# kjyv/FloBaRoID

Measured on AMD Instinct MI355X. Metric: regressor samples/s (fused regressor->Gram pass) + TSQR TFLOP/s, WALK-MAN 31-DOF float-base, higher is better.
Workload: dtype f64

## Files before the change

### flobaroid_amd/csrc/fbr_gram64.h

```cpp
#pragma once
#define FBR_G64_SWZ(c) (2 * ((c) & 15))
#include <algorithm>
#include <type_traits>
#include <utility>

#include "fbr_kinid.h"

struct FbrGram64Tile {
    int col[FBR_TILE];
    std::vector<int> path;
    int friction = 0;
    int lo = 0, hi = 0;
};

struct FbrGram64 {
    int NT = 0;
    int NF = 0;
    int nlev = 0, fb = 0, flev = 0, ntr = 0, maxact = 0, npw = 0, wpb = 8;
    long blk_doubles = 0;
    std::vector<int> trow;
    std::vector<int> slab;
    int nstage = 0, base_stages = 0;
    std::vector<int> stage_lev;
    std::vector<int> lev_begin;
// ... 661 lines not shown
        put(a, b, l[0], l[1], h[0], h[1]);
    }
    __device__ __forceinline__ double get8(double a) const { return dpp<0x128>(a); }
    __device__ __forceinline__ double get7(double a) const { return dpp<0x141>(a); }
    __device__ __forceinline__ double get2(double a) const { return dpp<0x4E>(a); }
    __device__ __forceinline__ double get1(double a) const { return dpp<0xB1>(a); }
    __device__ __forceinline__ double live0(bool live, double a) const { return live ? a : 0.0; }
    __device__ __forceinline__ double bit8(double a, double b) const { return (lane & 8) ? b : a; }
    __device__ __forceinline__ double zero() const { return 0.0; }
};

struct DevGram64 {
    int NT, nlev, maxact, npieces, nstage;
    long blk_doubles;
    const int *slab, *lev_begin, *pieces, *wmeta, *stage_lev;
    const int *runs;
};

template <int MAXD, bool HASW, int KR = 1>
__global__ __launch_bounds__(64 * FBR_KINWRITE_PARTS, MAXD <= 10 ? 2 : 1) void fbr_kinimg_kernel(DevModel m, DevKinId p, DevKinWrite wr, long S, long blk_doubles,
                                                                              const double *__restrict__ q, const double *__restrict__ dq,
                                                                              const double *__restrict__ ddq, const double *__restrict__ bv,
                                                                              const double *__restrict__ ba, const double *__restrict__ rpy,
                                                                              const double *__restrict__ rhs, const double *__restrict__ wts,
                                                                              double *__restrict__ scratch, double *__restrict__ mom,
                                                                              const double *__restrict__ sign)
{
    extern __shared__ __attribute__((aligned(16))) double smem[];
    const int lane = threadIdx.x & 63, part = __builtin_amdgcn_readfirstlane(threadIdx.x >> 6), nth = blockDim.x, tid = threadIdx.x;
    const int n = m.n, ldn = p.ldn, ldw = m.rows | 1, rows = m.rows;
    double *sq = smem, *sdq = sq + 64 * ldn, *sddq = sdq + 64 * ldn, *sw = sddq + 64 * ldn;
    double *st = sw + (HASW ? 64 * ldw : 0);
    double *scr = scratch + ((long)blockIdx.x * wr.nparts + part) * p.nslots * FBR_LINK_REC * 64 + lane;
    double *mo = mom ? mom + (long)blockIdx.x * (KR * wr.cols + KR * (KR + 1) / 2) : nullptr;
    const bool domom = KR > 1 || wr.k != 0;
    const FbrMomLanesDev mx{lane};
    const long Sg = wr.group_samples > 0 ? wr.group_samples : S, bpg = (Sg + 63) >> 6;
    const long nblk = (S / Sg) * bpg;
    const fbr_clong_ptr cdst = (fbr_clong_ptr)(unsigned long)wr.dst;
    const __attribute__((address_space(1))) int *glcol = (const __attribute__((address_space(1))) int *)(unsigned long)wr.lanecol + (long)part * m.L * 64 + lane;
    for (long blk = blockIdx.x; blk < nblk; blk += gridDim.x) {
        const long grp = blk / bpg, lb = blk - grp * bpg;
        const long base = grp * Sg + (lb << 6);
        const int valid = (int)min(64L, Sg - (lb << 6));
        __syncthreads();
        {
            const long off = base * n;
            const int cnt = valid * n;
            int sr = tid / n, dc = tid - sr * n;
            const int ds = nth / n, dd = nth - ds * n;
            for (int i = tid; i < cnt; i += nth) {
                const double a = q[off + i], b = dq[off + i], c = ddq[off + i];
                sq[sr * ldn + dc] = a;
                sdq[sr * ldn + dc] = b;
                sddq[sr * ldn + dc] = c;
                sr += ds;
                dc += dd;
                if (dc >= n) {
                    dc -= n;
                    sr++;
                }
            }
            if (HASW || wr.k) {
                const int cw = valid * rows;
                int wr_ = tid / rows, wc = tid - wr_ * rows;
                const int es = nth / rows, ed = nth - es * rows;
                for (int i = tid; i < cw; i += nth) {
                    const double wv = HASW ? wts[base * rows + i] : 1.0;
                    if (HASW) sw[wr_ * ldw + wc] = wv;
                    if constexpr (KR == 1) {
                        if (wr.k) st[wr_ * ldw + wc] = wv * wv * rhs[base * rows + i];
                    } else {
#pragma unroll
                        for (int r = 0; r < KR; r++) st[r * 64 * ldw + wr_ * ldw + wc] = wv * wv * rhs[(base * rows + i) * KR + r];
                    }
                    wr_ += es;
                    wc += ed;
                    if (wc >= rows) {
                        wc -= rows;
                        wr_++;
                    }
                }
            }
        }
        __syncthreads();
        const int ls = min(lane, valid - 1);
        const long s = base + ls;
        const bool live = lane < valid;
        const double *mysq = sq + ls * ldn, *mysdq = sdq + ls * ldn, *mysddq = sddq + ls * ldn, *myw = sw + ls * ldw, *myt = st + ls * ldw;
        const long slot_off = blk * blk_doubles + (long)(lane >> 5) * 512;
        const int s31 = lane & 31;
        auto state = [&](int d, double &a, double &b, double &c) {
            a = mysq[d];
            b = mysdq[d];
            c = mysddq[d];
        };
        auto basest = [&](double *v6, double *a6, double *e3) {
            for (int i = 0; i < 6; i++) {
                v6[i] = bv[s * 6 + i];
                a6[i] = ba[s * 6 + i];
            }
            for (int i = 0; i < 3; i++) e3[i] = rpy[s * 3 + i];
        };
        auto save = [&](int b, int i, double v) { scr[(b * FBR_LINK_REC + i) * 64] = v; };
        auto load = [&](int b, int i) { return scr[(b * FBR_LINK_REC + i) * 64]; };
        auto consts = [&](int l, double *rR, double *rp, double *ax) {
            const fbr_cdouble_ptr cR = (fbr_cdouble_ptr)(unsigned long)m.restR, cp = (fbr_cdouble_ptr)(unsigned long)m.restp,
                                  ca = (fbr_cdouble_ptr)(unsigned long)m.axis;
            for (int i = 0; i < 9; i++) rR[i] = cR[9 * l + i];
            for (int i = 0; i < 3; i++) {
                rp[i] = cp[3 * l + i];
                ax[i] = ca[3 * l + i];
            }
        };
        const unsigned vlane = (unsigned)(((unsigned long)slot_off + (unsigned long)s31) << 3);
        auto link = [&](int l, int depth, const double *rec, const double (*Sst)[6], const int *lvd, double *F) {
            (void)F;
            if (wr.base_only) depth = 0;
            if (wr.none && ((fbr_cint_ptr)(unsigned long)wr.none)[(long)part * m.L + l]) return;
            int mycol = -1;
            if (domom) mycol = glcol[l * 64];
            __builtin_amdgcn_s_waitcnt(0x0F70);
            double macc = 0.0;
            auto mom_sum = [&](auto g0c, auto ngc, auto p0c, auto nqc, const double *v, int r) {
                constexpr int G0 = decltype(g0c)::value, NG = decltype(ngc)::value, P0 = decltype(p0c)::value, NQ = decltype(nqc)::value;
                double u[NG];
#pragma unroll
                for (int i = 0; i < NG; i++) u[i] = (G0 + i >= P0 && G0 + i < P0 + NQ) ? v[G0 + i - P0] : 0.0;
                const double sum = fbr_mom_lanes_sum<NG>(u, live, mx);
                if (G0 == 0 ? (lane & 15) == 6 * r : (lane & 7) == 1 + 6 * r) macc += sum;
            };
            long d10[10], dF[4];
#pragma unroll
            for (int pp = 0; pp < 10; pp++) d10[pp] = cdst[((long)part * m.L + l) * FBR_G64_WORDS + pp];
#pragma unroll
            for (int pp = 0; pp < 4; pp++) dF[pp] = cdst[((long)part * m.L + l) * FBR_G64_WORDS + 10 + pp];
            auto ft_of = [&](int ro, double *F) {
#pragma unroll
                for (int i = 0; i < 6; i++)
                    if (i < m.fb) F[i] = myt[ro + i];
#pragma unroll
                for (int j = 0; j < MAXD; j++)
                    if (j < depth) {
                        const double tj = myt[ro + m.fb + lvd[j]];
#pragma unroll
                        for (int i = 0; i < 6; i++) F[i] += Sst[j][i] * tj;
                    }
            };
            double Ft[6] = {0.0, 0.0, 0.0, 0.0, 0.0, 0.0};
            if constexpr (KR == 1) {
                if (wr.k) {
#pragma unroll
                    for (int i = 0; i < 6; i++)
                        if (i < m.fb) Ft[i] = myt[i];
#pragma unroll
                    for (int j = 0; j < MAXD; j++)
                        if (j < depth) {
                            const double tj = myt[m.fb + lvd[j]];
#pragma unroll
                            for (int i = 0; i < 6; i++) Ft[i] += Sst[j][i] * tj;
                        }
                }
            }
            auto ft_group = [&](int r, double *F) {
                int ro = r * 64 * ldw;
                asm volatile("" : "+v"(ro));
#pragma unroll
                for (int i = 0; i < 6; i++) F[i] = 0.0;
                ft_of(ro, F);
// ... 72 lines not shown
                if (!domom || any == 0) return;
                double v[NQ];
                if constexpr (KR == 1) {
#pragma unroll
                    for (int qq = 0; qq < NQ; qq++) v[qq] = Ft[3] * nB[qq][0] + Ft[4] * nB[qq][1] + Ft[5] * nB[qq][2];
                    mom_sum(integral_constant<int, 4>{}, integral_constant<int, 6>{}, integral_constant<int, 4 + Q0>{}, nqc, v, 0);
                } else {
#pragma unroll
                    for (int r = 0; r < KR; r++) {
                        double F[6];
                        ft_group(r, F);
#pragma unroll
                        for (int qq = 0; qq < NQ; qq++) v[qq] = F[3] * nB[qq][0] + F[4] * nB[qq][1] + F[5] * nB[qq][2];
                        mom_sum(integral_constant<int, 4>{}, integral_constant<int, 6>{}, integral_constant<int, 4 + Q0>{}, nqc, v, r);
                    }
                }
            };
            if constexpr (MAXD > 8 && MAXD <= 10) {
                full_group(integral_constant<int, 0>{}, integral_constant<int, 2>{});
                full_group(integral_constant<int, 2>{}, integral_constant<int, 2>{});
                moment_group(integral_constant<int, 0>{}, integral_constant<int, 3>{});
                moment_group(integral_constant<int, 3>{}, integral_constant<int, 3>{});
            } else {
                full_group(integral_constant<int, 0>{}, integral_constant<int, 4>{});
                moment_group(integral_constant<int, 0>{}, integral_constant<int, 6>{});
            }
            const int nfr = wr.cols > wr.ninert ? (wr.cols - wr.ninert) / n : 0;
            const int dj = nfr ? m.dof[l] : -1;
            if (dj >= 0 && depth > 0) {
                const fbr_cint_ptr cfr = (fbr_cint_ptr)(unsigned long)(wr.lcol10 + (long)wr.nparts * 10 * m.L + ((long)part * m.L + l) * FBR_G64_FRIC);
#pragma unroll
                for (int pf = 0; pf < FBR_G64_FRIC; pf++)
                    if (pf < nfr) {
                        const long dfw = cdst[((long)part * m.L + l) * FBR_G64_WORDS + 14 + pf];
                        if (dfw == 0) continue;
                        const int c = cfr[pf];
                        const double fv = fbr_friction_value(m.coldesc[c].z, mysdq[dj], sign ? sign[s * n + dj] : 0.0, m.stribeck);
                        store(dfw, m.fb + depth - 1, HASW ? fv * myw[m.fb + dj] : fv);
                        if (!domom) continue;
#pragma unroll
                        for (int r = 0; r < KR; r++) {
                            const double v = fv * myt[r * 64 * ldw + m.fb + dj], sum = fbr_mom_lanes_sum<1>(&v, live, mx);
                            if (lane == fbr_gram64_mom_fric_lane(pf, r)) macc = sum;
                        }
                    }
            }
            if (domom && mycol >= 0 && (KR > 1 || mycol < (1 << FBR_G64_LANECOL_RHS)))
                unsafeAtomicAdd(mo + (mycol >> FBR_G64_LANECOL_RHS) * wr.cols + (mycol & ((1 << FBR_G64_LANECOL_RHS) - 1)), macc);
        };
        auto emit = [&](int, double) {};
        {
            fbr_kinid_lane<MAXD, false>(wr.part_nsteps[part], p.maxlvl, p.steps + wr.part_step0[part] * FBR_KINID_STEP, p.endflush, m.floating, m.g, m.fb,
                                        state, basest, save, load, link, emit, consts);
            if constexpr (KR == 1) {
                if (wr.k && part == wr.nparts - 1) {
                    double tt = 0.0;
                    for (int r = 0; r < rows; r++) {
                        const double wv = HASW ? myw[r] : 1.0, tv = rhs[s * rows + r] * wv;
                        tt += tv * tv;
                    }
                    const double sum = fbr_mom_lanes_sum<1>(&tt, live, mx);
                    if (lane == 0) unsafeAtomicAdd(mo + wr.cols, sum);
                }
            } else if (part == wr.nparts - 1) {
                double tt[KR * (KR + 1) / 2];
#pragma unroll
                for (int e = 0; e < KR * (KR + 1) / 2; e++) tt[e] = 0.0;
// ... 266 lines not shown
```

### flobaroid_amd/csrc/fbr_gram_api.hip

```cpp
#define FBR_KERNELS_GRAM
#include "fbr_internal.h"

static int get_deal(GramHolder *h, int wpg, GramHolder::Deal *out, bool base_only = false)
{
    const int key = wpg | (base_only ? 1 << 24 : 0);
    auto it = h->deals.find(key);
    if (it != h->deals.end()) {
        *out = it->second;
        return FBR_OK;
    }
    const std::vector<int> n = fbr_gram_deal(h->prog, wpg, base_only);
    std::vector<int2> tab;
    std::vector<int> begin(h->prog.T + 1, 0), given(h->prog.T, 0);
    for (int p = 0; p < h->prog.T; p++) begin[p + 1] = begin[p] + n[p];
    while ((int)tab.size() < begin[h->prog.T])
        for (int p = 0; p < h->prog.T; p++)
            if (given[p] < n[p]) tab.push_back(make_int2(p, given[p]++ | (n[p] << 16)));
    GramHolder::Deal d;
    int rc;
    if ((rc = upload(h->pool, tab, &d.tab))) return rc;
    if ((rc = upload(h->pool, begin, &d.begin))) return rc;
    h->deals[key] = d;
    *out = d;
    return FBR_OK;
// ... 250 lines not shown
{
    if (h->g64_state) return FBR_OK;
    h->g64_state = -1;
    const FbrHostModel &hm = m->hm;
    if (m->kinid.nsteps <= 0 || !fbr_gram64_build(hm, h->prog, h->g64, m->opt.gram_force_tiles != 0, m->opt.gram_lane_waves >= 16,
                                                         (int)m->opt.gram_lane_tiling))
        return FBR_OK;
    FbrGram64 &g = h->g64;
    if (fbr_gram64_lds_bytes(g) > FBR_G64_LDS_MAX) return FBR_OK;
    if (gram64_plds(hm, h->prog.k, true) > 160 * 1024) return FBR_OK;
    if (!fbr_gram64_build_producer(hm, g, h->g64p, m->opt.gram_lane_parts_cut != 0, h->prog.k)) return FBR_OK;
    std::vector<int> wgbegin{0, 0};
    int rc;
    if ((rc = upload(h->pool, g.slab, &h->d64_slab)) || (rc = upload(h->pool, g.lev_begin, &h->d64_levb)) || (rc = upload(h->pool, g.pieces, &h->d64_pieces)) ||
        (rc = upload(h->pool, g.wmeta, &h->d64_wmeta)) || (rc = upload(h->pool, h->g64p.lcol, &h->d64_lcol)) ||
        (rc = upload(h->pool, fbr_gram64_lane_columns(h->g64p, hm.L), &h->d64_lanecol)) ||
        (rc = upload(h->pool, h->g64p.steps, &h->d64_steps)) || (rc = upload(h->pool, h->g64p.none, &h->d64_none)) ||
        (rc = upload(h->pool, g.slot_tiles, &h->d64_slot_tiles)) || (rc = upload(h->pool, g.tilecol, &h->d64_tilecol)) ||
        (rc = upload(h->pool, g.stage_lev, &h->d64_stagelev)) || (!g.runs.empty() && (rc = upload(h->pool, g.runs, &h->d64_runs))))
        return rc;
    h->g64_state = 1;
    return FBR_OK;
}

static int gram64_serves(fbr_model *m, GramHolder *h, int k, bool *serves)
{
    *serves = false;
    if (!m->opt.gram_lane || k > FBR_G64_MAXK || (k > 0 && !h->moments)) return FBR_OK;
    if (int rc = get_gram64(m, h)) return rc;
    *serves = h->g64_state == 1;
    return FBR_OK;
}

static long gram64_chunk_blocks(const FbrGram64 &g) { return std::max<long>(1, (long)((size_t)3 * 1024 * 1024 * 1024 / ((size_t)g.blk_doubles * 8))); }

static int gram64_wg_table(GramHolder *h, int wgs, const int **out)
{
    auto it = h->d64_wb.find(wgs);
    if (it == h->d64_wb.end()) {
        std::vector<int> wb{0, wgs};
        const int *dwb = nullptr;
        if (int rc = upload(h->pool, wb, &dwb)) return rc;
        it = h->d64_wb.emplace(wgs, dwb).first;
    }
    *out = it->second;
    return FBR_OK;
}

static int gram64_ensure_images(fbr_model *m, GramHolder *h, long chb)
{
    const FbrGram64 &g = h->g64;
    int rc;
    if (chb <= h->img64_blocks) return FBR_OK;
    for (int b = 0; b < 2; b++) {
        if ((rc = h->img64[b].ensure((size_t)chb * g.blk_doubles * sizeof(double)))) return rc;
        HIPCHK(hipMemsetAsync(h->img64[b].p, 0, h->img64[b].bytes, m->stream));
        std::vector<long long> dst(h->g64p.rel.size(), 0);
        for (size_t i = 0; i < dst.size(); i++)
            if (h->g64p.rel[i]) dst[i] = (long long)(uintptr_t)h->img64[b].p + (h->g64p.rel[i] & ~(1LL << 62));
        if ((rc = h->dst64[b].ensure(dst.size() * sizeof(long long)))) return rc;
        HIPCHK(hipMemcpyAsync(h->dst64[b].p, dst.data(), dst.size() * sizeof(long long), hipMemcpyHostToDevice, m->stream));
        HIPCHK(hipStreamSynchronize(m->stream));
    }
    h->img64_blocks = chb;
    return FBR_OK;
}

template <class F> static auto kinimg_by_depth(const fbr_model *m, F &&f) { return fbr_by_depth<4, 8, 10, 12, FBR_KINID_MAXD>(m->kinid.maxlvl, f); }

struct Gram64Launch {
    DevKinId kp;
    int pgrid_max;
    DevGram64 dg;
    void (*gk)(DevGram64, long, const double *, double *, int);
    size_t glds;
    int vnpw;
};
static int gram64_setup(fbr_model *m, GramHolder *h, bool base_only, Gram64Launch *L)
{
    const FbrGram64 &g = h->g64;
    L->kp = kinid_params(m, 0, h->g64p.nslots, h->d64_steps);
    L->pgrid_max = kinimg_by_depth(m, [](auto D) { return D <= 10 ? 2 : 1; }) * m->num_cus;
    if (int rc = h->scr64.ensure((size_t)L->pgrid_max * h->g64p.nparts * std::max(h->g64p.nslots, 1) * FBR_LINK_REC * 64 * sizeof(double))) return rc;
    DevGram64 &dg = L->dg;
    dg.NT = g.NT + g.NF;
    dg.nlev = g.nlev;
    dg.maxact = g.maxact;
    dg.npieces = (int)g.pieces.size() / 2;
    dg.blk_doubles = g.blk_doubles;
    dg.slab = h->d64_slab;
    dg.lev_begin = h->d64_levb;
    dg.pieces = h->d64_pieces;
    dg.wmeta = h->d64_wmeta;
    dg.nstage = base_only ? g.base_stages : g.nstage;
    dg.stage_lev = h->d64_stagelev;
    dg.runs = g.runs.empty() ? nullptr : h->d64_runs;
    L->gk = g.wpb == 16 ? fbr_gram64_kernel<10, 16>
            : g.npw == 10   ? fbr_gram64_kernel<10, 8>
            : g.runs.empty() ? fbr_gram64_kernel<FBR_ONE_SEGW * FBR_ONE_NSEG, 8> : fbr_gram64_kernel<FBR_ONE_SEGW * FBR_ONE_NSEG, 8, true>;
    L->glds = fbr_gram64_lds_bytes(g);
    L->vnpw = g.npw * (g.wpb / 8);
    HIPCHK(hipFuncSetAttribute((const void *)L->gk, hipFuncAttributeMaxDynamicSharedMemorySize, (int)L->glds));
    return FBR_OK;
}

static DevKinWrite gram64_kinwrite(const fbr_model *m, const GramHolder *h, int b, int k, bool has_w, bool base_only, long group_samples)
{
    DevKinWrite kw{};
    kw.lcol10 = h->d64_lcol;
    kw.lanecol = h->d64_lanecol;
    kw.none = m->opt.gram_lane_skip_unowned != 0 ? h->d64_none : nullptr;
    kw.dst = (const long *)h->dst64[b].p;
    kw.ninert = m->hm.ninert;
    kw.cols = m->hm.cols;
    kw.k = k;
    kw.has_w = has_w ? 1 : 0;
    kw.flev = h->g64.flev;
    kw.base_only = base_only ? 1 : 0;
    kw.group_samples = group_samples;
    kw.nparts = h->g64p.nparts;
    for (int pq = 0; pq < FBR_KINWRITE_PARTS; pq++) {
        kw.part_nsteps[pq] = h->g64p.nsteps[pq];
        kw.part_step0[pq] = h->g64p.step0[pq];
    }
    return kw;
}

static int gram64_produce(fbr_model *m, GramHolder *h, const Gram64Launch &L, const DevKinWrite &kw, int pblocks, size_t plds, long cs,
                          const DevStates &d, long so, const double *rhs, int k, const double *w, double *mom)
{
    const FbrHostModel &hm = m->hm;
    return kinimg_by_depth(m, [&](auto D) -> int {
        const auto kernel = k == 2 ? (kw.has_w ? fbr_kinimg_kernel<D, true, 2> : fbr_kinimg_kernel<D, false, 2>)
                                   : (kw.has_w ? fbr_kinimg_kernel<D, true> : fbr_kinimg_kernel<D, false>);
        HIPCHK(hipFuncSetAttribute((const void *)kernel, hipFuncAttributeMaxDynamicSharedMemorySize, (int)plds));
        hipLaunchKernelGGL(kernel, dim3(pblocks), dim3(64 * h->g64p.nparts), plds, m->stream, m->dm, L.kp, kw, cs, h->g64.blk_doubles, d.q + so * hm.n,
                           d.dq + so * hm.n, d.ddq + so * hm.n, d.bv ? d.bv + so * 6 : nullptr, d.ba ? d.ba + so * 6 : nullptr,
                           d.rpy ? d.rpy + so * 3 : nullptr, rhs ? rhs + (size_t)so * hm.rows * k : nullptr, w ? w + (size_t)so * hm.rows : nullptr,
                           h->scr64.as<double>(), mom, d.sign ? d.sign + so * hm.n : nullptr);
        HIPCHK(hipGetLastError());
        return FBR_OK;
    });
}

static int gram64_reduce(fbr_model *m, GramHolder *h, const Gram64Launch &L, int wpg, const int *wg_begin, int ng, double *G)
// ... 30 lines not shown
        if (int rc = m->st_chunk[b].ensure(std::max<size_t>(1, (size_t)samples * per) * sizeof(double))) return rc;
    return FBR_OK;
}
static int stage_chunk(fbr_model *m, const DevStates &d, const double *rhs, int k, const double *w, long s0, long cs, int b, hipStream_t cps,
                       DevStates *dc, const double **crhs, const double **cw)
{
    const FbrHostModel &hm = m->hm;
    double *p = m->st_chunk[b].as<double>();
    auto put = [&](const double *src, size_t per, const double **dst) -> int {
        *dst = nullptr;
        if (!src || per == 0) return FBR_OK;
        HIPCHK(hipMemcpyAsync(p, src + (size_t)s0 * per, (size_t)cs * per * sizeof(double), hipMemcpyHostToDevice, cps));
        *dst = p;
        p += (size_t)cs * per;
        return FBR_OK;
    };
    *dc = d;
    int rc;
    if ((rc = put(d.q, hm.n, &dc->q)) || (rc = put(d.dq, hm.n, &dc->dq)) || (rc = put(d.ddq, hm.n, &dc->ddq)) || (rc = put(d.bv, 6, &dc->bv)) ||
        (rc = put(d.ba, 6, &dc->ba)) || (rc = put(d.rpy, 3, &dc->rpy)) || (rc = put(d.sign, hm.n, &dc->sign)) ||
        (rc = put(rhs, (size_t)hm.rows * k, crhs)) || (rc = put(w, hm.rows, cw)))
        return rc;
    return FBR_OK;
}

static int gram64_pass(fbr_model *m, GramHolder *h, const DevStates &d, const double *drhs, const double *dw, int k, double *G, bool base_only,
                       bool h2d_chunked)
{
    const FbrHostModel &hm = m->hm;
    const FbrGram64 &g = h->g64;
    const long S = d.S;
    int rc;
    const long nblocks = (S + 63) / 64;
    long chb = gram64_chunk_blocks(g);
    if (h2d_chunked) chb = std::min<long>(chb, 7L * m->num_cus);
    if (m->opt.chunk_samples >= 1) chb = std::min(gram64_chunk_blocks(g), std::max<long>(1, ((long)m->opt.chunk_samples + 63) / 64));
    chb = std::min(nblocks, chb);
    if (chb < nblocks && chb > m->num_cus) chb = chb / m->num_cus * m->num_cus;
    Gram64Launch L;
    if ((rc = gram64_setup(m, h, base_only, &L))) return rc;
    long last_blocks = 0;
    if (m->opt.gram_lane_chunk_rounds != 0 && !h2d_chunked && m->opt.chunk_samples < 1 && chb < nblocks && chb >= m->num_cus) {
        const FbrGram64ChunkPlan cp = fbr_gram64_chunk_plan(nblocks, gram64_chunk_blocks(g), m->num_cus, L.pgrid_max, 1);
        chb = cp.chb;
        last_blocks = cp.last_cap;
    }
    long chs = chb * 64;
    if (m->opt.chunk_samples >= 1) chs = std::min(chs, (long)m->opt.chunk_samples);
    const long last_s = last_blocks > 0 ? last_blocks * 64 : chs;
    auto chunk_len = [&](long s0) { return S - s0 <= last_s ? S - s0 : chs; };
    if ((rc = gram64_ensure_images(m, h, std::min(nblocks, std::max(chb, last_blocks))))) return rc;
    const size_t plds = gram64_plds(hm, k, dw != nullptr);
    const int pblocks = (int)std::min<long>(chb, (long)L.pgrid_max);
    const int gwgs = (int)std::min<long>(chb, (long)m->num_cus);
    if (k) {
        if ((rc = h->mom64.ensure((size_t)L.pgrid_max * fbr_gram64_mom_count(hm.cols, k) * sizeof(double)))) return rc;
        HIPCHK(hipMemsetAsync(h->mom64.p, 0, (size_t)pblocks * fbr_gram64_mom_count(hm.cols, k) * sizeof(double), m->stream));
    }
    if ((rc = m->partial.ensure((size_t)m->num_cus * g.wpb * g.npw * 256 * sizeof(double)))) return rc;
    int launches = 0, first_wgs = 0;
    if (h2d_chunked) {
        if ((rc = ensure_stage_buffers(m, d, k, dw, chs, 2)) || (rc = ensure_copy_stream(m))) return rc;
        HIPCHK(hipEventRecord(m->ev_fork, m->stream));
    }
    struct Staged {
        DevStates dc;
        long o;
        const double *rhs, *w;
    };
    auto stage = [&](long c, Staged &out) -> int {
        const long s0 = c * chs, cs = chunk_len(s0);
        const int b = (int)(c & 1);
        out = {d, s0, drhs, dw};
        if (!h2d_chunked) return FBR_OK;
        HIPCHK(hipStreamWaitEvent(m->copy, m->ev_pack_rec[b] ? m->ev_pack[b] : m->ev_fork, 0));
        ProfScope ps(m, FBR_PROF_H2D, m->copy);
        if (int r3 = stage_chunk(m, d, drhs, k, dw, s0, cs, b, m->copy, &out.dc, &out.rhs, &out.w)) return r3;
        out.o = 0;
        HIPCHK(hipEventRecord(m->ev_h2d[b], m->copy));
        return FBR_OK;
    };
    Staged cur, nxt;
    if (S > 0 && (rc = stage(0, nxt))) return rc;
    for (long s0 = 0, cs = 0; s0 < S; s0 += cs, launches++) {
        cs = chunk_len(s0);
        const long nb = (cs + 63) / 64;
        const int b = launches & 1;
        cur = nxt;
        if (s0 + cs < S && (rc = stage(launches + 1, nxt))) return rc;
        if (h2d_chunked) HIPCHK(hipStreamWaitEvent(m->stream, m->ev_h2d[b], 0));
        {
            ProfScope ps(m, FBR_PROF_PACK);
            if ((rc = gram64_produce(m, h, L, gram64_kinwrite(m, h, b, k, dw != nullptr, base_only, 0), pblocks, plds, cs, cur.dc, cur.o, cur.rhs, k,
                                     cur.w, k ? h->mom64.as<double>() : nullptr)))
                return rc;
            if (cs & 63) {
                hipLaunchKernelGGL(fbr_gram64_tail_zero_kernel, dim3(16, 1), dim3(256), 0, m->stream, h->img64[b].as<double>(), g.blk_doubles, nb, g.ntr, (int)(cs & 63));
                HIPCHK(hipGetLastError());
            }
            if (h2d_chunked) {
                HIPCHK(hipEventRecord(m->ev_pack[b], m->stream));
                m->ev_pack_rec[b] = true;
            }
        }
        const int wgs = (int)std::min<long>(nb, (long)gwgs);
        if (launches == 0) first_wgs = wgs;
        if (wgs > first_wgs) {
            set_err("internal: Gram launch wider than the first one of the call");
            return FBR_E_INVALID;
        }
        {
            ProfScope ps(m, FBR_PROF_GRAM);
            hipLaunchKernelGGL(L.gk, dim3(first_wgs), dim3(g.wpb * 64), L.glds, m->stream, L.dg, nb, h->img64[b].as<double>(), m->partial.as<double>(),
                               launches > 0 ? 1 : 0);
            HIPCHK(hipGetLastError());
        }
    }
    if (launches > 0) {
        ProfScope ps(m, FBR_PROF_REDUCE);
        const int *wgb = nullptr;
        if ((rc = gram64_wg_table(h, first_wgs, &wgb)) || (rc = gram64_reduce(m, h, L, first_wgs, wgb, 1, G))) return rc;
        if (k) {
            hipLaunchKernelGGL(fbr_gram64_mom_reduce_kernel, dim3((fbr_gram64_mom_count(hm.cols, k) + 3) / 4), dim3(256), 0, m->stream, hm.cols, k, pblocks,
                               h->mom64.as<double>(), G);
            HIPCHK(hipGetLastError());
        }
    }
    return FBR_OK;
}

static int gram64_grouped_pass(fbr_model *m, GramHolder *h, const DevStates &d, const double *dw, double *G, int ngroups)
{
    const FbrHostModel &hm = m->hm;
    const FbrGram64 &g = h->g64;
    const long S = d.S, Sg = S / ngroups, bpg = (Sg + 63) / 64;
    const int Pa = hm.cols;
    int rc;
    const int gpc = (int)std::min<long>(std::min(ngroups, 32768), std::max<long>(1, gram64_chunk_blocks(g) / bpg));
    if ((rc = gram64_ensure_images(m, h, (long)gpc * bpg))) return rc;
    const int wpg = (int)std::max<long>(1, std::min<long>(bpg, (long)m->num_cus / std::min(gpc, ngroups)));
    Gram64Launch L;
    if ((rc = gram64_setup(m, h, false, &L))) return rc;
    const size_t plds = gram64_plds(hm, 0, dw != nullptr);
    if ((rc = m->partial.ensure((size_t)gpc * wpg * g.wpb * g.npw * 256 * sizeof(double)))) return rc;
    const int *wgb = nullptr;
    if ((rc = gram64_wg_table(h, wpg, &wgb))) return rc;
    for (int g0 = 0, launches = 0; g0 < ngroups; g0 += gpc, launches++) {
        const int ng = std::min(gpc, ngroups - g0), b = launches & 1;
        const long s0 = (long)g0 * Sg, cs = (long)ng * Sg, nb = (long)ng * bpg;
        {
            ProfScope ps(m, FBR_PROF_PACK);
            if ((rc = gram64_produce(m, h, L, gram64_kinwrite(m, h, b, 0, dw != nullptr, false, Sg), (int)std::min<long>(nb, (long)L.pgrid_max), plds, cs,
                                     d, s0, nullptr, 0, dw, nullptr)))
                return rc;
            if (Sg & 63) {
                hipLaunchKernelGGL(fbr_gram64_tail_zero_kernel, dim3(16, ng), dim3(256), 0, m->stream, h->img64[b].as<double>(), g.blk_doubles, bpg, g.ntr, (int)(Sg & 63));
                HIPCHK(hipGetLastError());
            }
        }
        {
            ProfScope ps(m, FBR_PROF_GRAM);
            hipLaunchKernelGGL(L.gk, dim3(wpg, ng), dim3(g.wpb * 64), L.glds, m->stream, L.dg, bpg, h->img64[b].as<double>(), m->partial.as<double>(), 0);
            HIPCHK(hipGetLastError());
        }
        {
            ProfScope ps(m, FBR_PROF_REDUCE);
            if ((rc = gram64_reduce(m, h, L, wpg, wgb, ng, G + (size_t)g0 * Pa * Pa))) return rc;
        }
    }
    return FBR_OK;
}

static int print_gram_timing(fbr_model *m, int T, const unsigned long long *dbg, int NW)
{
    std::vector<unsigned long long> hb((size_t)NW * FBR_WPB * 8);
    HIPCHK(hipMemcpyAsync(hb.data(), dbg, hb.size() * sizeof(unsigned long long), hipMemcpyDeviceToHost, m->stream));
    HIPCHK(hipStreamSynchronize(m->stream));
    static const char *names[3] = {"wait_dma+barrier", "dma_issue", "mfma"};
    std::vector<double> sum((size_t)T * 3, 0.0), ns(T, 0.0), nw(T, 0.0), wv((size_t)T * FBR_WPB, 0.0);
    for (size_t e = 0; e + 8 <= hb.size(); e += 8) {
        const int part = (int)hb[e + 6];
        if (part < 0 || part >= T) continue;
        for (int i = 0; i < 3; i++) sum[(size_t)part * 3 + i] += (double)hb[e + i];
        ns[part] += (double)hb[e + 7];
        nw[part] += 1.0;
        wv[(size_t)part * FBR_WPB + (e / 8) % FBR_WPB] += (double)hb[e + 2];
    }
    for (int part = 0; part < T; part++) {
        fprintf(stderr, "[fbr gram timing] part %d (cycles per sample per wave):", part);
        for (int i = 0; i < 3; i++) fprintf(stderr, " %s=%.0f", names[i], sum[(size_t)part * 3 + i] / std::max(ns[part], 1.0));
        fprintf(stderr, " | workgroups=%.0f cycles per workgroup=%.0f | mfma phase per wave:", nw[part] / FBR_WPB,
                (sum[(size_t)part * 3] + sum[(size_t)part * 3 + 1] + sum[(size_t)part * 3 + 2]) / std::max(nw[part], 1.0));
        for (int w = 0; w < FBR_WPB; w++) fprintf(stderr, " %.0f", wv[(size_t)part * FBR_WPB + w] * FBR_WPB / std::max(ns[part], 1.0));
        fprintf(stderr, "\n");
    }
// ... 210 lines not shown
        dw = w;
    } else {
        if ((rc = stage_one(m, m->st_aux, rhs, (size_t)S * hm.rows * k, st->mem, &drhs))) return rc;
        if ((rc = stage_one(m, m->st_aux2, w, (size_t)S * hm.rows, st->mem, &dw))) return rc;
    }
    bool base_only = false;
    if (w && S > 0 && hm.fb > 0 && hm.rows > hm.fb) {
        if (st->mem == FBR_HOST) {
            base_only = true;
            for (long s = 0; s < S && base_only; s++)
                for (int r = hm.fb; r < hm.rows; r++)
                    if (w[s * hm.rows + r] != 0.0) {
                        base_only = false;
                        break;
                    }
        } else {
            std::vector<char> act;
            if ((rc = active_rows(m, dw, S, &act))) return rc;
            base_only = true;
            for (int r = hm.fb; r < hm.rows; r++) base_only = base_only && !act[r];
        }
    }
    double *G = G_out;
    if (out_mem == FBR_HOST) {
        if ((rc = m->g_tmp.ensure(gcount * sizeof(double)))) return rc;
        G = m->g_tmp.as<double>();
        if (accumulate) HIPCHK(hipMemcpyAsync(G, G_out, gcount * sizeof(double), hipMemcpyHostToDevice, m->stream));
    }
    if (!accumulate) HIPCHK(hipMemsetAsync(G, 0, gcount * sizeof(double), m->stream));
    bool lane = false;
    if (S > 0 && d.q && !m->opt.gram_timing && !m->opt.gram_serial && (ngroups == 1 || (k == 0 && !h2d_chunked && !base_only)) &&
        (rc = gram64_serves(m, h, k, &lane)))
        return rc;
    if (lane && ngroups > 1 && (S / ngroups + 63) / 64 <= gram64_chunk_blocks(h->g64))
        rc = gram64_grouped_pass(m, h, d, dw, G, ngroups);
    else if (lane && ngroups == 1)
        rc = gram64_pass(m, h, d, drhs, dw, k, G, base_only && h->g64.base_stages > 0, h2d_chunked);
    else if (S > 0)
        rc = gram_image_pass(m, h, d, drhs, dw, k, G, ngroups, base_only, h2d_chunked, overlap_prev, async);
    if (rc) return rc;
    if (S > 0 && !async && h2d_chunked && m->copy) HIPCHK(hipStreamSynchronize(m->copy));
    if (async) {
        const int64_t t = m->next_ticket++;
        m->ticket_kind[t & 1] = 0;
        m->last_submit_kind = 0;
        HIPCHK(hipEventRecord(m->ev_done[t & 1], m->stream));
        *async_ticket = t;
        return FBR_OK;
    }
    return finish_output(m, G, G_out, gcount, out_mem);
}

static int gram_impl(fbr_model *m, const fbr_states *st, const double *rhs, int32_t k, const double *w, double *G_out, int32_t out_mem,
                     int32_t accumulate, int32_t ngroups, int64_t *async_ticket);

static int gram_via_red(fbr_model *m, int which, const fbr_states *st, const double *rhs, int32_t k, const double *w, double *G_out, int32_t out_mem,
                        int32_t accumulate, int32_t ngroups, int64_t *async_ticket)
{
    fbr_model *r = m->rdm[which].get();
    const bool async = async_ticket != nullptr;
    int rc;
    if ((rc = enter(m))) return rc;
    if ((rc = wait_ticket(m, async ? m->next_ticket - 2 : m->next_ticket - 1))) return rc;
    if (async && out_mem != FBR_DEVICE) {
        set_err("fbr_gram_submit takes a device-resident output and device-resident or PINNED host states / rhs / weights");
        return FBR_E_INVALID;
    }
// ... 84 lines not shown
```

### flobaroid_amd/csrc/fbr_internal.h

```cpp
#pragma once
#include <hip/hip_runtime.h>
#include <unistd.h>

#include <algorithm>
#include <cstdint>
#include <cstdio>
#include <cstdlib>
#include <cstring>
#include <map>
#include <memory>
#include <numeric>
#include <string>
#include <vector>

#include "../../include/fbr.h"
#include "fbr_options.h"
#include "fbr_kernels.h"
#include "fbr_kinid.h"
#include "fbr_capsule.h"
#include "fbr_capsule_grad.h"
#include "fbr_box.h"
#include "fbr_box_grad.h"
#include "fbr_hull.h"
#include "fbr_hull_grad.h"
// ... 128 lines not shown
        meshes = FBR_MESHES_NONE;
        geo = DevMeshes{0, nullptr, nullptr, nullptr, nullptr, nullptr, nullptr};
        bvh = DevMeshBvh{nullptr, nullptr, nullptr};
    }
    void clear()
    {
        clear_meshes();
        set = kNoHulls;
        grad = DevPairGrad{0, nullptr, nullptr};
        host = {};
        large_set = false;
        big = -1, big_nv = 0;
        views = FbrHullViews{};
    }
};

struct GramHolder {
    FbrGramProgram prog;
    DevGram dev;
    std::vector<DevBuf> pool;
    DevBuf pimg[2];
    bool moments = false;
    DevBuf mom[2];
    bool mom_clean[2] = {false, false};
    const int *itemcol = nullptr;
    size_t lds_bytes = 0;
    size_t pack_lds_bytes = 0;
    int g64_state = 0;
    FbrGram64 g64;
    FbrGram64Producer g64p;
    const int *d64_slab = nullptr, *d64_levb = nullptr, *d64_pieces = nullptr, *d64_wmeta = nullptr, *d64_lcol = nullptr, *d64_lanecol = nullptr, *d64_none = nullptr,
              *d64_steps = nullptr, *d64_slot_tiles = nullptr, *d64_tilecol = nullptr, *d64_stagelev = nullptr,
              *d64_runs = nullptr;
    DevBuf img64[2], dst64[2], mom64, scr64;
    long img64_blocks = 0;
    std::map<int, const int *> d64_wb;
    struct Deal { const int2 *tab; const int *begin; };
    std::map<int, Deal> deals;
};

struct fbr_model {
    FbrOptions opt;
    FbrHostModel hm;
    DevModel dm;
    int device = 0;
    pid_t pid = 0;
    int num_cus = 256;
    hipStream_t own_stream = nullptr, stream = nullptr;
    hipStream_t side = nullptr;
    hipStream_t copy = nullptr;
    hipEvent_t ev_pack[2] = {nullptr, nullptr}, ev_gram[2] = {nullptr, nullptr}, ev_fork = nullptr, ev_h2d[2] = {nullptr, nullptr};
    hipEvent_t ev_done[2] = {nullptr, nullptr};
    int64_t next_ticket = 0;
    int64_t waited_ticket = -1;
    bool submitting = false;
    bool ev_gram_rec[2] = {false, false};
    bool ev_pack_rec[2] = {false, false};
    DevBuf rec2;
    std::vector<DevBuf> tables;
    std::map<int, std::unique_ptr<GramHolder>> gram;
    DevBuf st_q, st_dq, st_ddq, st_bv, st_ba, st_rpy, st_sign, st_aux, st_aux2, st_x;
    DevBuf rec, partial, out_tmp, g_tmp;
    DevBuf st_chunk[2];
    DevBuf fd[7];
    DevBuf row_flags;
    FbrKinIdProgram kinid;
    const int *kinid_steps = nullptr, *kinid_endflush = nullptr;
// ... 165 lines not shown
```

### flobaroid_amd/csrc/fbr_kinid.h

```cpp
#pragma once
#include <type_traits>
#include <vector>

#include "fbr_math.h"
#include "fbr_program.h"

#define FBR_KINID_STEP 8
#define FBR_KINID_MAXD 24

#define FBR_KINWRITE_PARTS 4

#define FBR_SUSP_REC 39
#define FBR_SUSP_I 0
#define FBR_SUSP_B 6
#define FBR_SUSP_C0 15
#define FBR_SUSP_MC 18
#define FBR_SUSP_R 21
#define FBR_SUSP_P 30
#define FBR_SUSP_V 33

template <int D, int... Ds, class F> inline auto fbr_by_depth(int maxlvl, F &&f)
{
    if constexpr (sizeof...(Ds) > 0)
        if (maxlvl > D) return fbr_by_depth<Ds...>(maxlvl, f);
// ... 222 lines not shown
}

#if defined(__HIPCC__)
struct DevKinId {
    int nsteps, maxlvl, nslots, ldn;
    const int *steps, *endflush;
};
struct DevKinExt {
    long T, tiles, nblk;
    double *val;
    long *idx;
};
FBR_HD double fbr_ext_value(int k, double v)
{
    if (k == 2) return fabs(v);
    if (k == 3) return v != v ? 0.0 : fmin(fabs(v), 1.7976931348623157e308);
    return v;
}
FBR_HD bool fbr_ext_take(int k, double a, double b)
{
    if (b != b) return false;
    return a != a || (k == 0 ? a < b : a > b);
}
typedef __attribute__((address_space(1))) char *fbr_gchar_ptr;
typedef __attribute__((address_space(1))) double *fbr_gdouble_ptr;
struct DevKinWrite {
    const int *lcol10, *colrec;
    const int *lanecol = nullptr;
    const long *dst;
    int ninert, cols, k, has_w;
    int flev;
    int base_only;
    long group_samples;
    const int *none = nullptr;
    int nparts, part_nsteps[FBR_KINWRITE_PARTS], part_step0[FBR_KINWRITE_PARTS];
};
#endif

#if defined(__HIPCC__) && defined(FBR_KERNELS_CORE)

__device__ __forceinline__ double fbr_friction_std(const DevModel &m, const double *__restrict__ x, int d, double dqv, double sg, const double *vs)
{
    const int n = m.n;
    double t = sg * x[m.fstart + d];
    if (!m.grav_only) {
        t += x[m.fstart + n + d] * dqv;
        const int poff = m.fstart + 2 * n;
        t += x[poff + d];
        if (m.stribeck > 0) {
            const double sgn = (sg > 0) - (sg < 0);
            t += x[poff + n + d] * exp(-fabs(*vs) / m.stribeck) * sgn;
        }
    }
    return t;
}

template <int MAXD, bool EXT = false>
__global__ __launch_bounds__(64) void fbr_kinid_kernel(DevModel m, DevKinId p, long S, const double *__restrict__ q, const double *__restrict__ dq,
                                                       const double *__restrict__ ddq, const double *__restrict__ bv,
                                                       const double *__restrict__ ba, const double *__restrict__ rpy,
                                                       const double *__restrict__ sign, const double *__restrict__ vel_sign,
                                                       const double *__restrict__ x, int mode, double *__restrict__ tau, double *__restrict__ scratch, int flink, double fpx,
                                                       double fpy, double fpz, DevKinExt ex)
{
    extern __shared__ __attribute__((aligned(16))) double smem[];
    const int lane = threadIdx.x, n = m.n, ldn = p.ldn;
// ... 811 lines not shown
```

### flobaroid_amd/csrc/fbr_options.h

```cpp
#pragma once
#include <cstring>

struct FbrOptions {
    double link_merge = 1;
    double regroup = 1;
    double reduce_min_work = 1e9;
    double reduce_grouped_min_samples = 512;
    double chunk_samples = 0;
    double min_chunks = 4;
    double h2d_chunked = 1;
    double fused_id = 1;
    double hull_large_all = 0;
    double hull_grad_tile = 0;
    double mesh_grad_order = 0;
    double gram_lane_waves = 8;
    double gram_force_tiles = 1;
    double gram_lane = 1;
    double gram_lane_tiling = 1;
    double gram_lane_skip_unowned = 1;
    double gram_lane_parts_cut = 0;
    double gram_lane_chunk_rounds = 0;
    double gram_shape = 0;
    double gram_rhs_tile = 0;
    double gram_orient = 1;
    double gram_serial = 0;
    double gram_timing = 0;
    double tsqr_groups = 1;
    double tsqr_group_min_samples = 24000;
    double tsqr_reorder = 1;
    double tsqr_tree_one_wg = 0;
    double tsqr_narrow = 1;
    double tsqr_narrow_tall = 1;
    double tsqr_force_group = 1;
    double tsqr_lane_writer = 1;
    double tsqr_writer = 0;
    double tsqr_side_trees_beside = 0;
    double tsqr_prologue_overlap = 1;
    double tsqr_timing = 0;
    double tsqr_short_call_factors = 1;
};

struct FbrOptionKey {
    const char *name;
    double FbrOptions::*field;
    bool rebuild_programs;
};

static inline const FbrOptionKey *fbr_option_keys(int *count)
{
    static const FbrOptionKey keys[] = {
        {"link_merge", &FbrOptions::link_merge, false},
        {"regroup", &FbrOptions::regroup, false},
        {"reduce_min_work", &FbrOptions::reduce_min_work, false},
        {"reduce_grouped_min_samples", &FbrOptions::reduce_grouped_min_samples, false},
        {"chunk_samples", &FbrOptions::chunk_samples, false},
        {"min_chunks", &FbrOptions::min_chunks, false},
        {"h2d_chunked", &FbrOptions::h2d_chunked, false},
        {"fused_id", &FbrOptions::fused_id, false},
        {"hull_large_all", &FbrOptions::hull_large_all, false},
        {"hull_grad_tile", &FbrOptions::hull_grad_tile, false},
        {"mesh_grad_order", &FbrOptions::mesh_grad_order, false},
        {"gram_lane", &FbrOptions::gram_lane, false},
        {"gram_force_tiles", &FbrOptions::gram_force_tiles, true},
        {"gram_lane_waves", &FbrOptions::gram_lane_waves, true},
        {"gram_lane_tiling", &FbrOptions::gram_lane_tiling, true},
        {"gram_lane_skip_unowned", &FbrOptions::gram_lane_skip_unowned, true},
        {"gram_lane_parts_cut", &FbrOptions::gram_lane_parts_cut, true},
        {"gram_lane_chunk_rounds", &FbrOptions::gram_lane_chunk_rounds, true},
        {"gram_shape", &FbrOptions::gram_shape, true},
        {"gram_rhs_tile", &FbrOptions::gram_rhs_tile, true},
        {"gram_orient", &FbrOptions::gram_orient, true},
        {"gram_serial", &FbrOptions::gram_serial, false},
        {"gram_timing", &FbrOptions::gram_timing, false},
        {"tsqr_groups", &FbrOptions::tsqr_groups, false},
        {"tsqr_group_min_samples", &FbrOptions::tsqr_group_min_samples, false},
        {"tsqr_reorder", &FbrOptions::tsqr_reorder, false},
        {"tsqr_tree_one_wg", &FbrOptions::tsqr_tree_one_wg, false},
        {"tsqr_narrow", &FbrOptions::tsqr_narrow, false},
        {"tsqr_narrow_tall", &FbrOptions::tsqr_narrow_tall, false},
        {"tsqr_lane_writer", &FbrOptions::tsqr_lane_writer, false},
        {"tsqr_force_group", &FbrOptions::tsqr_force_group, false},
        {"tsqr_writer", &FbrOptions::tsqr_writer, false},
        {"tsqr_side_trees_beside", &FbrOptions::tsqr_side_trees_beside, false},
        {"tsqr_prologue_overlap", &FbrOptions::tsqr_prologue_overlap, false},
        {"tsqr_timing", &FbrOptions::tsqr_timing, false},
        {"tsqr_short_call_factors", &FbrOptions::tsqr_short_call_factors, false},
    };
    *count = (int)(sizeof(keys) / sizeof(keys[0]));
    return keys;
}

static inline const FbrOptionKey *fbr_option_find(const char *name)
{
    int n = 0;
    const FbrOptionKey *k = fbr_option_keys(&n);
    for (int i = 0; i < n; i++)
        if (name && !strcmp(k[i].name, name)) return &k[i];
    return nullptr;
}
```

Measured before the change: 89.33 million.

## Replace double-buffered Gram images with one larger image and per-block offsets

The two ping-pong image buffers and their destination-pointer tables become a single image of configurable size, by default 6 GiB instead of 3 GiB per buffer. Destination words now hold offsets from the chunk base, and the block base is added inside the kernel. A moment-slot rotation (mom_shift) is added so successive chunks accumulate into different per-block moment slots. The aim is fewer, larger chunks and fewer launches, at the cost of losing any overlap between producing one chunk and reducing the previous one.

```diff
diff --git a/flobaroid_amd/csrc/fbr_gram64.h b/flobaroid_amd/csrc/fbr_gram64.h
--- a/flobaroid_amd/csrc/fbr_gram64.h
+++ b/flobaroid_amd/csrc/fbr_gram64.h
@@ -717,7 +717,7 @@
     double *sq = smem, *sdq = sq + 64 * ldn, *sddq = sdq + 64 * ldn, *sw = sddq + 64 * ldn;
     double *st = sw + (HASW ? 64 * ldw : 0);
     double *scr = scratch + ((long)blockIdx.x * wr.nparts + part) * p.nslots * FBR_LINK_REC * 64 + lane;
-    double *mo = mom ? mom + (long)blockIdx.x * (KR * wr.cols + KR * (KR + 1) / 2) : nullptr;
+    double *mo = mom ? mom + (long)((blockIdx.x + wr.mom_shift) % gridDim.x) * (KR * wr.cols + KR * (KR + 1) / 2) : nullptr;
     const bool domom = KR > 1 || wr.k != 0;
     const FbrMomLanesDev mx{lane};
     const long Sg = wr.group_samples > 0 ? wr.group_samples : S, bpg = (Sg + 63) >> 6;
@@ -773,7 +773,7 @@
         const long s = base + ls;
         const bool live = lane < valid;
         const double *mysq = sq + ls * ldn, *mysdq = sdq + ls * ldn, *mysddq = sddq + ls * ldn, *myw = sw + ls * ldw, *myt = st + ls * ldw;
-        const long slot_off = blk * blk_doubles + (long)(lane >> 5) * 512;
+        const long blk_base = blk * blk_doubles * 8;
         const int s31 = lane & 31;
         auto state = [&](int d, double &a, double &b, double &c) {
             a = mysq[d];
@@ -798,7 +798,11 @@
                 ax[i] = ca[3 * l + i];
             }
         };
-        const unsigned vlane = (unsigned)(((unsigned long)slot_off + (unsigned long)s31) << 3);
+        const unsigned vlane = (unsigned)(((lane >> 5) * 512 + s31) << 3);
+        auto word = [&](long i) {
+            const long w = cdst[i];
+            return w ? w + blk_base : 0L;
+        };
         auto link = [&](int l, int depth, const double *rec, const double (*Sst)[6], const int *lvd, double *F) {
             (void)F;
             if (wr.base_only) depth = 0;
@@ -817,9 +821,9 @@
             };
             long d10[10], dF[4];
 #pragma unroll
-            for (int pp = 0; pp < 10; pp++) d10[pp] = cdst[((long)part * m.L + l) * FBR_G64_WORDS + pp];
-#pragma unroll
-            for (int pp = 0; pp < 4; pp++) dF[pp] = cdst[((long)part * m.L + l) * FBR_G64_WORDS + 10 + pp];
+            for (int pp = 0; pp < 10; pp++) d10[pp] = word(((long)part * m.L + l) * FBR_G64_WORDS + pp);
+#pragma unroll
+            for (int pp = 0; pp < 4; pp++) dF[pp] = word(((long)part * m.L + l) * FBR_G64_WORDS + 10 + pp);
             auto ft_of = [&](int ro, double *F) {
 #pragma unroll
                 for (int i = 0; i < 6; i++)
@@ -958,7 +962,7 @@
 #pragma unroll
                 for (int pf = 0; pf < FBR_G64_FRIC; pf++)
                     if (pf < nfr) {
-                        const long dfw = cdst[((long)part * m.L + l) * FBR_G64_WORDS + 14 + pf];
+                        const long dfw = word(((long)part * m.L + l) * FBR_G64_WORDS + 14 + pf);
                         if (dfw == 0) continue;
                         const int c = cfr[pf];
                         const double fv = fbr_friction_value(m.coldesc[c].z, mysdq[dj], sign ? sign[s * n + dj] : 0.0, m.stribeck);
diff --git a/flobaroid_amd/csrc/fbr_gram_api.hip b/flobaroid_amd/csrc/fbr_gram_api.hip
--- a/flobaroid_amd/csrc/fbr_gram_api.hip
+++ b/flobaroid_amd/csrc/fbr_gram_api.hip
@@ -306,7 +306,10 @@
     return FBR_OK;
 }
 
-static long gram64_chunk_blocks(const FbrGram64 &g) { return std::max<long>(1, (long)((size_t)3 * 1024 * 1024 * 1024 / ((size_t)g.blk_doubles * 8))); }
+static long gram64_chunk_blocks(const fbr_model *m, const FbrGram64 &g)
+{
+    return std::max<long>(1, (long)((size_t)std::max(m->opt.gram_lane_image_bytes, 0.0) / ((size_t)g.blk_doubles * 8)));
+}
 
 static int gram64_wg_table(GramHolder *h, int wgs, const int **out)
 {
@@ -326,16 +329,14 @@
     const FbrGram64 &g = h->g64;
     int rc;
     if (chb <= h->img64_blocks) return FBR_OK;
-    for (int b = 0; b < 2; b++) {
-        if ((rc = h->img64[b].ensure((size_t)chb * g.blk_doubles * sizeof(double)))) return rc;
-        HIPCHK(hipMemsetAsync(h->img64[b].p, 0, h->img64[b].bytes, m->stream));
-        std::vector<long long> dst(h->g64p.rel.size(), 0);
-        for (size_t i = 0; i < dst.size(); i++)
-            if (h->g64p.rel[i]) dst[i] = (long long)(uintptr_t)h->img64[b].p + (h->g64p.rel[i] & ~(1LL << 62));
-        if ((rc = h->dst64[b].ensure(dst.size() * sizeof(long long)))) return rc;
-        HIPCHK(hipMemcpyAsync(h->dst64[b].p, dst.data(), dst.size() * sizeof(long long), hipMemcpyHostToDevice, m->stream));
-        HIPCHK(hipStreamSynchronize(m->stream));
-    }
+    if ((rc = h->img64.ensure((size_t)chb * g.blk_doubles * sizeof(double)))) return rc;
+    HIPCHK(hipMemsetAsync(h->img64.p, 0, h->img64.bytes, m->stream));
+    std::vector<long long> dst(h->g64p.rel.size(), 0);
+    for (size_t i = 0; i < dst.size(); i++)
+        if (h->g64p.rel[i]) dst[i] = (long long)(uintptr_t)h->img64.p + (h->g64p.rel[i] & ~(1LL << 62));
+    if ((rc = h->dst64.ensure(dst.size() * sizeof(long long)))) return rc;
+    HIPCHK(hipMemcpyAsync(h->dst64.p, dst.data(), dst.size() * sizeof(long long), hipMemcpyHostToDevice, m->stream));
+    HIPCHK(hipStreamSynchronize(m->stream));
     h->img64_blocks = chb;
     return FBR_OK;
 }
@@ -378,13 +379,13 @@
     return FBR_OK;
 }
 
-static DevKinWrite gram64_kinwrite(const fbr_model *m, const GramHolder *h, int b, int k, bool has_w, bool base_only, long group_samples)
+static DevKinWrite gram64_kinwrite(const fbr_model *m, const GramHolder *h, int k, bool has_w, bool base_only, long group_samples)
 {
     DevKinWrite kw{};
     kw.lcol10 = h->d64_lcol;
     kw.lanecol = h->d64_lanecol;
     kw.none = m->opt.gram_lane_skip_unowned != 0 ? h->d64_none : nullptr;
-    kw.dst = (const long *)h->dst64[b].p;
+    kw.dst = (const long *)h->dst64.p;
     kw.ninert = m->hm.ninert;
     kw.cols = m->hm.cols;
     kw.k = k;
@@ -481,16 +482,16 @@
     const long S = d.S;
     int rc;
     const long nblocks = (S + 63) / 64;
-    long chb = gram64_chunk_blocks(g);
+    long chb = gram64_chunk_blocks(m, g);
     if (h2d_chunked) chb = std::min<long>(chb, 7L * m->num_cus);
-    if (m->opt.chunk_samples >= 1) chb = std::min(gram64_chunk_blocks(g), std::max<long>(1, ((long)m->opt.chunk_samples + 63) / 64));
+    if (m->opt.chunk_samples >= 1) chb = std::min(gram64_chunk_blocks(m, g), std::max<long>(1, ((long)m->opt.chunk_samples + 63) / 64));
     chb = std::min(nblocks, chb);
     if (chb < nblocks && chb > m->num_cus) chb = chb / m->num_cus * m->num_cus;
     Gram64Launch L;
     if ((rc = gram64_setup(m, h, base_only, &L))) return rc;
     long last_blocks = 0;
     if (m->opt.gram_lane_chunk_rounds != 0 && !h2d_chunked && m->opt.chunk_samples < 1 && chb < nblocks && chb >= m->num_cus) {
-        const FbrGram64ChunkPlan cp = fbr_gram64_chunk_plan(nblocks, gram64_chunk_blocks(g), m->num_cus, L.pgrid_max, 1);
+        const FbrGram64ChunkPlan cp = fbr_gram64_chunk_plan(nblocks, gram64_chunk_blocks(m, g), m->num_cus, L.pgrid_max, 1);
         chb = cp.chb;
         last_blocks = cp.last_cap;
     }
@@ -508,6 +509,7 @@
     }
     if ((rc = m->partial.ensure((size_t)m->num_cus * g.wpb * g.npw * 256 * sizeof(double)))) return rc;
     int launches = 0, first_wgs = 0;
+    long blocks_done = 0;
     if (h2d_chunked) {
         if ((rc = ensure_stage_buffers(m, d, k, dw, chs, 2)) || (rc = ensure_copy_stream(m))) return rc;
         HIPCHK(hipEventRecord(m->ev_fork, m->stream));
@@ -540,11 +542,12 @@
         if (h2d_chunked) HIPCHK(hipStreamWaitEvent(m->stream, m->ev_h2d[b], 0));
         {
             ProfScope ps(m, FBR_PROF_PACK);
-            if ((rc = gram64_produce(m, h, L, gram64_kinwrite(m, h, b, k, dw != nullptr, base_only, 0), pblocks, plds, cs, cur.dc, cur.o, cur.rhs, k,
-                                     cur.w, k ? h->mom64.as<double>() : nullptr)))
-                return rc;
+            DevKinWrite kw = gram64_kinwrite(m, h, k, dw != nullptr, base_only, 0);
+            kw.mom_shift = (int)(blocks_done % pblocks);
+            blocks_done += nb;
+            if ((rc = gram64_produce(m, h, L, kw, pblocks, plds, cs, cur.dc, cur.o, cur.rhs, k, cur.w, k ? h->mom64.as<double>() : nullptr))) return rc;
             if (cs & 63) {
-                hipLaunchKernelGGL(fbr_gram64_tail_zero_kernel, dim3(16, 1), dim3(256), 0, m->stream, h->img64[b].as<double>(), g.blk_doubles, nb, g.ntr, (int)(cs & 63));
+                hipLaunchKernelGGL(fbr_gram64_tail_zero_kernel, dim3(16, 1), dim3(256), 0, m->stream, h->img64.as<double>(), g.blk_doubles, nb, g.ntr, (int)(cs & 63));
                 HIPCHK(hipGetLastError());
             }
             if (h2d_chunked) {
@@ -560,7 +563,7 @@
         }
         {
             ProfScope ps(m, FBR_PROF_GRAM);
-            hipLaunchKernelGGL(L.gk, dim3(first_wgs), dim3(g.wpb * 64), L.glds, m->stream, L.dg, nb, h->img64[b].as<double>(), m->partial.as<double>(),
+            hipLaunchKernelGGL(L.gk, dim3(first_wgs), dim3(g.wpb * 64), L.glds, m->stream, L.dg, nb, h->img64.as<double>(), m->partial.as<double>(),
                                launches > 0 ? 1 : 0);
             HIPCHK(hipGetLastError());
         }
@@ -585,7 +588,7 @@
     const long S = d.S, Sg = S / ngroups, bpg = (Sg + 63) / 64;
     const int Pa = hm.cols;
     int rc;
-    const int gpc = (int)std::min<long>(std::min(ngroups, 32768), std::max<long>(1, gram64_chunk_blocks(g) / bpg));
+    const int gpc = (int)std::min<long>(std::min(ngroups, 32768), std::max<long>(1, gram64_chunk_blocks(m, g) / bpg));
     if ((rc = gram64_ensure_images(m, h, (long)gpc * bpg))) return rc;
     const int wpg = (int)std::max<long>(1, std::min<long>(bpg, (long)m->num_cus / std::min(gpc, ngroups)));
     Gram64Launch L;
@@ -594,22 +597,22 @@
     if ((rc = m->partial.ensure((size_t)gpc * wpg * g.wpb * g.npw * 256 * sizeof(double)))) return rc;
     const int *wgb = nullptr;
     if ((rc = gram64_wg_table(h, wpg, &wgb))) return rc;
-    for (int g0 = 0, launches = 0; g0 < ngroups; g0 += gpc, launches++) {
-        const int ng = std::min(gpc, ngroups - g0), b = launches & 1;
+    for (int g0 = 0; g0 < ngroups; g0 += gpc) {
+        const int ng = std::min(gpc, ngroups - g0);
         const long s0 = (long)g0 * Sg, cs = (long)ng * Sg, nb = (long)ng * bpg;
         {
             ProfScope ps(m, FBR_PROF_PACK);
-            if ((rc = gram64_produce(m, h, L, gram64_kinwrite(m, h, b, 0, dw != nullptr, false, Sg), (int)std::min<long>(nb, (long)L.pgrid_max), plds, cs,
+            if ((rc = gram64_produce(m, h, L, gram64_kinwrite(m, h, 0, dw != nullptr, false, Sg), (int)std::min<long>(nb, (long)L.pgrid_max), plds, cs,
                                      d, s0, nullptr, 0, dw, nullptr)))
                 return rc;
             if (Sg & 63) {
-                hipLaunchKernelGGL(fbr_gram64_tail_zero_kernel, dim3(16, ng), dim3(256), 0, m->stream, h->img64[b].as<double>(), g.blk_doubles, bpg, g.ntr, (int)(Sg & 63));
+                hipLaunchKernelGGL(fbr_gram64_tail_zero_kernel, dim3(16, ng), dim3(256), 0, m->stream, h->img64.as<double>(), g.blk_doubles, bpg, g.ntr, (int)(Sg & 63));
                 HIPCHK(hipGetLastError());
             }
         }
         {
             ProfScope ps(m, FBR_PROF_GRAM);
-            hipLaunchKernelGGL(L.gk, dim3(wpg, ng), dim3(g.wpb * 64), L.glds, m->stream, L.dg, bpg, h->img64[b].as<double>(), m->partial.as<double>(), 0);
+            hipLaunchKernelGGL(L.gk, dim3(wpg, ng), dim3(g.wpb * 64), L.glds, m->stream, L.dg, bpg, h->img64.as<double>(), m->partial.as<double>(), 0);
             HIPCHK(hipGetLastError());
         }
         {
@@ -886,7 +889,7 @@
     if (S > 0 && d.q && !m->opt.gram_timing && !m->opt.gram_serial && (ngroups == 1 || (k == 0 && !h2d_chunked && !base_only)) &&
         (rc = gram64_serves(m, h, k, &lane)))
         return rc;
-    if (lane && ngroups > 1 && (S / ngroups + 63) / 64 <= gram64_chunk_blocks(h->g64))
+    if (lane && ngroups > 1 && (S / ngroups + 63) / 64 <= gram64_chunk_blocks(m, h->g64))
         rc = gram64_grouped_pass(m, h, d, dw, G, ngroups);
     else if (lane && ngroups == 1)
         rc = gram64_pass(m, h, d, drhs, dw, k, G, base_only && h->g64.base_stages > 0, h2d_chunked);
diff --git a/flobaroid_amd/csrc/fbr_internal.h b/flobaroid_amd/csrc/fbr_internal.h
--- a/flobaroid_amd/csrc/fbr_internal.h
+++ b/flobaroid_amd/csrc/fbr_internal.h
@@ -184,7 +184,7 @@
     const int *d64_slab = nullptr, *d64_levb = nullptr, *d64_pieces = nullptr, *d64_wmeta = nullptr, *d64_lcol = nullptr, *d64_lanecol = nullptr, *d64_none = nullptr,
               *d64_steps = nullptr, *d64_slot_tiles = nullptr, *d64_tilecol = nullptr, *d64_stagelev = nullptr,
               *d64_runs = nullptr;
-    DevBuf img64[2], dst64[2], mom64, scr64;
+    DevBuf img64, dst64, mom64, scr64;
     long img64_blocks = 0;
     std::map<int, const int *> d64_wb;
     struct Deal { const int2 *tab; const int *begin; };
diff --git a/flobaroid_amd/csrc/fbr_kinid.h b/flobaroid_amd/csrc/fbr_kinid.h
--- a/flobaroid_amd/csrc/fbr_kinid.h
+++ b/flobaroid_amd/csrc/fbr_kinid.h
@@ -278,6 +278,7 @@
     int flev;
     int base_only;
     long group_samples;
+    int mom_shift = 0;
     const int *none = nullptr;
     int nparts, part_nsteps[FBR_KINWRITE_PARTS], part_step0[FBR_KINWRITE_PARTS];
 };
diff --git a/flobaroid_amd/csrc/fbr_options.h b/flobaroid_amd/csrc/fbr_options.h
--- a/flobaroid_amd/csrc/fbr_options.h
+++ b/flobaroid_amd/csrc/fbr_options.h
@@ -20,6 +20,7 @@
     double gram_lane_skip_unowned = 1;
     double gram_lane_parts_cut = 0;
     double gram_lane_chunk_rounds = 0;
+    double gram_lane_image_bytes = 6442450944.0;
     double gram_shape = 0;
     double gram_rhs_tile = 0;
     double gram_orient = 1;
@@ -67,6 +68,7 @@
         {"gram_lane_skip_unowned", &FbrOptions::gram_lane_skip_unowned, true},
         {"gram_lane_parts_cut", &FbrOptions::gram_lane_parts_cut, true},
         {"gram_lane_chunk_rounds", &FbrOptions::gram_lane_chunk_rounds, true},
+        {"gram_lane_image_bytes", &FbrOptions::gram_lane_image_bytes, false},
         {"gram_shape", &FbrOptions::gram_shape, true},
         {"gram_rhs_tile", &FbrOptions::gram_rhs_tile, true},
         {"gram_orient", &FbrOptions::gram_orient, true},
```

After: 90.77 million (median of 6 runs). 1.02x the previous value.
